# ZhenghaoFei/visual_odom

Measured on NVIDIA B200. Metric: stereo frames/sec at 1241x376, 2000 feats; LK kernel HBM GB/s vs roofline, higher is better.
Workload: dtype u8/i32 fixed point + f32 (LK), f64 (pose)

## Files before the change

### visual_odom_b200/csrc/batch.cu

```cuda
#include "ctx.h"
#include <string.h>

__global__ void k_pack_counts(vo_unit_result_dev* res, const int* n_pts, const int* n_det, const int* n3, const int* n5,
                              int n_units, int detect)
{
    const int u = blockIdx.x * blockDim.x + threadIdx.x;
    if (u >= n_units) return;
    res[u].n_features = n_pts[u];
    res[u].n_detected = detect ? n_det[u] : 0;
    res[u].n_tracked = n3[u];
    res[u].n_valid = n5[u];
}

#define VO_OUT_BYTES_PER_SLOT (4 * sizeof(float2) + sizeof(int) + sizeof(float3) + sizeof(int))
__global__ void k_pack_outputs(uint8_t* __restrict__ out, size_t stride, int per, const float2* __restrict__ valid4, size_t cs,
                               const int* __restrict__ idx5, const float3* __restrict__ X, const int* __restrict__ inliers,
                               const int* __restrict__ n5, const vo_unit_result_dev* __restrict__ res, int cap)
{
    const int u = blockIdx.x;
    const int nv = min(n5[u], per), ni = min(res[u].n_inliers, per);
    float2* o4 = reinterpret_cast<float2*>(out + (size_t)u * stride);
    int* ok = reinterpret_cast<int*>(o4 + 4 * (size_t)per);
    float* oX = reinterpret_cast<float*>(ok + per);
    int* oi = reinterpret_cast<int*>(oX + 3 * (size_t)per);
// ... 125 lines not shown
    return VO_OK;
}

static int ensure_hi_streams(vo_ctx* ctx)
{
    if (ctx->hi_stream[0]) return VO_OK;
    int lo = 0, hi = 0;
    VO_CUDA_CHECK(cudaDeviceGetStreamPriorityRange(&lo, &hi));
    for (int c = 0; c < VO_LANES; c++) {
        VO_CUDA_CHECK(cudaStreamCreateWithPriority(&ctx->hi_stream[c], cudaStreamNonBlocking, hi));
        for (int k = 0; k < 4; k++) VO_CUDA_CHECK(cudaEventCreateWithFlags(&ctx->hi_ev[c][k], cudaEventDisableTiming));
    }
    return VO_OK;
}

static int run_range_launch(vo_ctx* ctx, const View& v)
{
    ctx->imgs_per_unit = 4;
    int rc;
    int c = -1;
    for (int k = 0; k < VO_LANES; k++) if (ctx->side_stream[k] && v.s == ctx->side_stream[k]) c = k;
    const bool part = ctx->part_on && c >= 0;
    const bool prio = !part && ctx->use_priorities && c >= 0;
    View h = v, lk = v;
    cudaEvent_t* ev = nullptr;
    if (part) {
        h.s = ctx->part_hp_stream[c]; lk.s = ctx->part_lk_stream[c]; ev = ctx->part_ev[c];
    } else if (prio) {
        if ((rc = ensure_hi_streams(ctx))) return rc;
        h.s = ctx->hi_stream[c]; ev = ctx->hi_ev[c];
    }
    View pre = h;
    if (part && ctx->part_pre_with_lk) pre.s = lk.s;
    if (ev) {
        VO_CUDA_CHECK(cudaEventRecord(ev[0], v.s));
        VO_CUDA_CHECK(cudaStreamWaitEvent(pre.s, ev[0], 0));
        if (pre.s != h.s) VO_CUDA_CHECK(cudaStreamWaitEvent(h.s, ev[0], 0));
    }
    if (ctx->batch_detect) {
        if ((rc = vo_run_fast(ctx, pre, 0, false))) return rc;
        if ((rc = vo_run_select(ctx, pre))) return rc;
    }
    if ((rc = vo_run_pyramid(ctx, v.u0 * ctx->imgs_per_unit, v.n * ctx->imgs_per_unit, pre.s))) return rc;
    if (ev && pre.s != lk.s) {
        VO_CUDA_CHECK(cudaEventRecord(ev[1], pre.s));
        VO_CUDA_CHECK(cudaStreamWaitEvent(lk.s, ev[1], 0));
    }
    const int ip[4] = {0, 1, 3, 2}, in[4] = {1, 3, 2, 0};
    ctx->lk_per_unit = ctx->batch_max_pts;
    rc = vo_run_lk_ring(ctx, lk, 4, ip, in, false);
    ctx->lk_per_unit = 0;
    if (rc) return rc;
    if (ev) {
        VO_CUDA_CHECK(cudaEventRecord(ev[2], lk.s));
        VO_CUDA_CHECK(cudaStreamWaitEvent(h.s, ev[2], 0));
    }
    if ((rc = vo_run_filter(ctx, h, false))) return rc;
    const size_t cs = (size_t)ctx->units * ctx->cap;
    if ((rc = vo_run_triangulate(ctx, h, ctx->d_valid4, ctx->d_valid4 + cs, ctx->d_n5))) return rc;
    float K9[9] = {ctx->P_l[0], ctx->P_l[1], ctx->P_l[2], ctx->P_l[4], ctx->P_l[5], ctx->P_l[6], ctx->P_l[8], ctx->P_l[9], ctx->P_l[10]};
    if ((rc = vo_run_pnp(ctx, h, ctx->d_valid4 + 2 * cs, ctx->d_n5, K9))) return rc;
    k_pack_counts<<<(v.n + 63) / 64, 64, 0, h.s>>>(ctx->d_results + v.u0, ctx->d_npts + v.u0, ctx->d_ndet + v.u0, ctx->d_n3 + v.u0,
                                                  ctx->d_n5 + v.u0, v.n, ctx->batch_detect ? 1 : 0);
    ctx->launches += 1;
    VO_CUDA_CHECK(cudaGetLastError());
    if (ev) {
        VO_CUDA_CHECK(cudaEventRecord(ev[3], h.s));
        VO_CUDA_CHECK(cudaStreamWaitEvent(v.s, ev[3], 0));
    }
    return VO_OK;
}

static int run_range(vo_ctx* ctx, const View& v)
{
    bool on_side = false;
    for (int k = 0; k < VO_LANES; k++) on_side = on_side || (ctx->side_stream[k] && v.s == ctx->side_stream[k]);
// ... 237 lines not shown
```

### visual_odom_b200/csrc/ctx.cu

```cuda
#include "ctx.h"
#include <string.h>
#include <stdlib.h>

void vo_set_error(vo_ctx* ctx, const char* fmt, ...)
{
    if (!ctx) return;
    va_list ap;
    va_start(ap, fmt);
    vsnprintf(ctx->err, sizeof(ctx->err), fmt, ap);
    va_end(ap);
}

extern "C" void vo_default_params(vo_params* p)
{
    p->fast_threshold = 20;
    p->fast_nonmax = 1;
    p->lk_win = 21;
    p->lk_max_level = 3;
    p->lk_max_iters = 30;
    p->lk_epsilon = 0.01;
    p->lk_min_eig = 0.001;
    p->circ_threshold = 0;
    p->pnp_iterations = 500;
    p->pnp_reproj_error = 0.5f;
// ... 155 lines not shown
    if (!allow_pending_batches)
        for (auto& p : ctx->pending)
            if (p.active) {
                vo_set_error(ctx, "%s: the vo_batch_submit submission of slots [%d, %d) has not been waited for", who, p.u0, p.u0 + p.n);
                return VO_E_INVALID;
            }
    ctx->seq_active = false;
    return VO_OK;
}

typedef CUresult (*PFN_cuDeviceGet)(CUdevice*, int);
typedef CUresult (*PFN_cuDeviceGetDevResource)(CUdevice, CUdevResource*, CUdevResourceType);
typedef CUresult (*PFN_cuDevSmResourceSplitByCount)(CUdevResource*, unsigned int*, const CUdevResource*, CUdevResource*, unsigned int, unsigned int);
typedef CUresult (*PFN_cuDevResourceGenerateDesc)(CUdevResourceDesc*, CUdevResource*, unsigned int);
typedef CUresult (*PFN_cuGreenCtxCreate)(CUgreenCtx*, CUdevResourceDesc, CUdevice, unsigned int);
typedef CUresult (*PFN_cuGreenCtxStreamCreate)(CUstream*, CUgreenCtx, unsigned int, int);
typedef CUresult (*PFN_cuGreenCtxDestroy)(CUgreenCtx);

template <typename F>
static bool drv(const char* name, F* fn)
{
    void* p = nullptr;
    cudaDriverEntryPointQueryResult q;
    if (cudaGetDriverEntryPoint(name, &p, cudaEnableDefault, &q) != cudaSuccess || q != cudaDriverEntryPointSuccess || !p) return false;
    *fn = (F)p;
    return true;
}

void vo_partition_destroy(vo_ctx* ctx)
{
    for (int c = 0; c < VO_LANES; c++) {
        if (ctx->part_lk_stream[c]) cudaStreamDestroy(ctx->part_lk_stream[c]);
        if (ctx->part_hp_stream[c]) cudaStreamDestroy(ctx->part_hp_stream[c]);
        ctx->part_lk_stream[c] = ctx->part_hp_stream[c] = nullptr;
        for (int k = 0; k < 4; k++) if (ctx->part_ev[c][k]) { cudaEventDestroy(ctx->part_ev[c][k]); ctx->part_ev[c][k] = nullptr; }
    }
    PFN_cuGreenCtxDestroy destroy = nullptr;
    if (drv("cuGreenCtxDestroy", &destroy))
        for (int k = 0; k < 2; k++) if (ctx->part_gctx[k]) destroy((CUgreenCtx)ctx->part_gctx[k]);
    ctx->part_gctx[0] = ctx->part_gctx[1] = nullptr;
    ctx->part_on = false; ctx->part_helper_sms = ctx->part_lk_sms = 0;
}

int vo_partition_enable(vo_ctx* ctx, int helper_sms)
{
    VO_CUDA_CHECK(cudaSetDevice(ctx->device));
    int rc = vo_drain_pending(ctx);
    if (rc) return rc;
    VO_CUDA_CHECK(cudaDeviceSynchronize());
    vo_drop_graphs(ctx);
    vo_partition_destroy(ctx);
    if (helper_sms <= 0) return VO_OK;
    PFN_cuDeviceGet dget; PFN_cuDeviceGetDevResource getres; PFN_cuDevSmResourceSplitByCount split;
    PFN_cuDevResourceGenerateDesc gendesc; PFN_cuGreenCtxCreate create; PFN_cuGreenCtxStreamCreate screate;
    if (!drv("cuDeviceGet", &dget) || !drv("cuDeviceGetDevResource", &getres) || !drv("cuDevSmResourceSplitByCount", &split) ||
        !drv("cuDevResourceGenerateDesc", &gendesc) || !drv("cuGreenCtxCreate", &create) || !drv("cuGreenCtxStreamCreate", &screate)) {
        vo_set_error(ctx, "sm_partition: this driver has no green-context API");
        return VO_E_UNSUPPORTED;
    }
    CUdevice dev;
    CUdevResource all, part[1], rest;
    unsigned int nb = 1;
    CUresult r;
    if ((r = dget(&dev, ctx->device)) != CUDA_SUCCESS || (r = getres(dev, &all, CU_DEV_RESOURCE_TYPE_SM)) != CUDA_SUCCESS ||
        (r = split(part, &nb, &all, &rest, 0, (unsigned)helper_sms)) != CUDA_SUCCESS || nb != 1) {
        vo_set_error(ctx, "sm_partition: splitting off %d SMs failed (driver error %d)", helper_sms, (int)r);
        return VO_E_UNSUPPORTED;
    }
    CUdevResource* rs[2] = {&part[0], &rest};
    for (int k = 0; k < 2; k++) {
        CUdevResourceDesc desc;
        CUgreenCtx g;
        if ((r = gendesc(&desc, rs[k], 1)) != CUDA_SUCCESS || (r = create(&g, desc, dev, CU_GREEN_CTX_DEFAULT_STREAM)) != CUDA_SUCCESS) {
            vo_set_error(ctx, "sm_partition: cuGreenCtxCreate failed (driver error %d)", (int)r);
            vo_partition_destroy(ctx);
            return VO_E_UNSUPPORTED;
        }
        ctx->part_gctx[k] = g;
    }
    ctx->part_helper_sms = (int)part[0].sm.smCount; ctx->part_lk_sms = (int)rest.sm.smCount;
    for (int c = 0; c < VO_LANES; c++) {
        CUstream a, b;
        if ((r = screate(&a, (CUgreenCtx)ctx->part_gctx[0], CU_STREAM_NON_BLOCKING, 0)) != CUDA_SUCCESS ||
            (r = screate(&b, (CUgreenCtx)ctx->part_gctx[1], CU_STREAM_NON_BLOCKING, 0)) != CUDA_SUCCESS) {
            vo_set_error(ctx, "sm_partition: cuGreenCtxStreamCreate failed (driver error %d)", (int)r);
            vo_partition_destroy(ctx);
            return VO_E_UNSUPPORTED;
        }
        ctx->part_hp_stream[c] = (cudaStream_t)a; ctx->part_lk_stream[c] = (cudaStream_t)b;
        for (int k = 0; k < 4; k++) VO_CUDA_CHECK(cudaEventCreateWithFlags(&ctx->part_ev[c][k], cudaEventDisableTiming));
    }
    ctx->part_on = true;
    return VO_OK;
}

int vo_drain_pending(vo_ctx* ctx)
{
    for (auto& p : ctx->pending)
        if (p.active) {
            VO_CUDA_CHECK(cudaEventSynchronize(p.done));
            p.active = false;
        }
    if (ctx->seq_inflight > 0 && ctx->side_stream[0]) VO_CUDA_CHECK(cudaStreamSynchronize(ctx->side_stream[0]));
    return VO_OK;
}

void vo_drop_graphs(vo_ctx* ctx)
{
    for (auto& g : ctx->graphs) cudaGraphExecDestroy(g.exec);
    ctx->graphs.clear();
}

void vo_set_calibration(vo_ctx* ctx, const float P_l[12], const float P_r[12])
{
    const bool same = ctx->have_P && memcmp(ctx->P_l, P_l, 12 * sizeof(float)) == 0 && memcmp(ctx->P_r, P_r, 12 * sizeof(float)) == 0;
    if (same) return;
    vo_drop_graphs(ctx);
    memcpy(ctx->P_l, P_l, 12 * sizeof(float));
    memcpy(ctx->P_r, P_r, 12 * sizeof(float));
    ctx->have_P = true;
}

void vo_free_state(vo_ctx* ctx)
// ... 235 lines not shown
        for (int c = 0; c < VO_LANES; c++) if (ctx->part_on && v.s == ctx->part_lk_stream[c]) lk_sms = ctx->part_lk_sms;
        VO_CUDA_CHECK(vo_launch_lk_ring(ctx->maps, a, lk_sms, ctx->lk_ctas_per_sm, v.s));
    }
    ctx->launches += 1;
    if (e1) VO_CUDA_CHECK(cudaEventRecord(e1, v.s));
    return VO_OK;
}

int vo_run_filter(vo_ctx* ctx, const View& v, bool with_ages)
{
    const size_t uo = (size_t)v.u0 * ctx->cap;
    FilterArgs f;
    memset(&f, 0, sizeof(f));
    f.cap = ctx->cap;
    f.call_stride = (size_t)ctx->units * ctx->cap;
    f.circ_threshold = ctx->p.circ_threshold;
    f.n_pts = ctx->d_npts + v.u0;
    f.pts_in = ctx->d_pts_in + uo;
    f.pts_out = ctx->d_pts_out + uo;
    f.status = ctx->d_status + uo;
    f.ages_in = with_ages ? ctx->d_ages_in + uo : nullptr;
    f.ages_out = ctx->d_ages_out + uo;
    f.kept5 = ctx->d_kept5 + uo;
    f.idx3 = ctx->d_idx3 + uo;
    f.n3 = ctx->d_n3 + v.u0;
    f.valid4 = ctx->d_valid4 + uo;
    f.idx5 = ctx->d_idx5 + uo;
    f.n5 = ctx->d_n5 + v.u0;
    VO_CUDA_CHECK(vo_launch_ring_filter(f, v.n, v.s));
    ctx->launches += 1;
    return VO_OK;
}

int vo_run_fast(vo_ctx* ctx, const View& v, int plane_in_unit, bool want_resp)
{
    FastArgs a;
    memset(&a, 0, sizeof(a));
    const size_t plane = (size_t)ctx->w * ctx->h;
    a.n_units = v.n;
    a.img_tab = ctx->d_raw_tab + (size_t)(v.plane0 >= 0 ? v.plane0 : v.u0 * ctx->imgs_per_unit) + plane_in_unit;
    a.img_stride_idx = ctx->imgs_per_unit;
    a.w = ctx->w; a.h = ctx->h; a.pitch = ctx->w;
    a.threshold = ctx->p.fast_threshold; a.nonmax = ctx->p.fast_nonmax;
    a.score = ctx->d_score + v.u0 * plane; a.score_plane = plane;
    a.rowbuf = ctx->d_rowbuf + v.u0 * plane; a.rowcap = ctx->w;
    a.rowcount = ctx->d_rowcount + (size_t)v.u0 * ctx->h; a.rowoff = ctx->d_rowoff + (size_t)v.u0 * ctx->h;
    a.n_det = ctx->d_ndet + v.u0;
    a.corners = ctx->d_corners + (size_t)v.u0 * ctx->corner_cap;
    a.resp = want_resp ? ctx->d_resp + (size_t)v.u0 * ctx->corner_cap : nullptr;
    a.corner_cap = ctx->corner_cap;
    ctx->launches += vo_launch_fast(a, v.s);
    VO_CUDA_CHECK(cudaGetLastError());
    return VO_OK;
}

int vo_run_select(vo_ctx* ctx, const View& v)
{
    ctx->launches += vo_launch_select(ctx->d_corners + (size_t)v.u0 * ctx->corner_cap, ctx->corner_cap, ctx->d_ndet + v.u0,
                                      ctx->d_want + v.u0, ctx->d_pts_in + (size_t)v.u0 * ctx->cap, ctx->cap, ctx->d_npts + v.u0,
                                      v.n, v.s);
    VO_CUDA_CHECK(cudaGetLastError());
    return VO_OK;
}

int vo_run_triangulate(vo_ctx* ctx, const View& v, const float2* pts_l, const float2* pts_r, const int* n, float4* X4)
{
    const size_t uo = (size_t)v.u0 * ctx->cap;
    TriArgs t;
    memset(&t, 0, sizeof(t));
    t.cap = ctx->cap; t.n_pts = n + v.u0; t.pts_l = pts_l + uo; t.pts_r = pts_r + uo; t.X = ctx->d_X + uo; t.X4 = X4;
    for (int k = 0; k < 12; k++) { t.Pl[k] = (double)ctx->P_l[k]; t.Pr[k] = (double)ctx->P_r[k]; }
    ctx->launches += vo_launch_triangulate(t, v.n, v.s);
    VO_CUDA_CHECK(cudaGetLastError());
    return VO_OK;
}

int vo_run_pnp(vo_ctx* ctx, const View& v, const float2* pts2d, const int* n, const float* K9)
{
    const size_t uo = (size_t)v.u0 * ctx->cap, its = (size_t)ctx->p.pnp_iterations;
    PnpArgs a;
    memset(&a, 0, sizeof(a));
    a.n_units = v.n; a.cap = ctx->cap; a.iterations = ctx->p.pnp_iterations;
    a.n_pts = n + v.u0; a.X = ctx->d_X + uo; a.x = pts2d + uo;
    a.fu = (double)K9[0]; a.fv = (double)K9[4]; a.uc = (double)K9[2]; a.vc = (double)K9[5];
    const double thr = (double)ctx->p.pnp_reproj_error;
    a.thr2 = (float)(thr * thr);
    a.confidence = ctx->p.pnp_confidence;
    a.t_prev = ctx->d_tprev + (size_t)v.u0 * 3;
    a.state = ctx->d_pnp_state + v.u0; a.subsets = ctx->d_subsets + v.u0 * its * 5; a.models = ctx->d_models + v.u0 * its * 12;
    a.counts = ctx->d_counts + v.u0 * its;
    a.inliers = ctx->d_inliers + uo; a.results = ctx->d_results + v.u0;
    ctx->launches += vo_launch_pnp(a, v.s);
    VO_CUDA_CHECK(cudaGetLastError());
    return VO_OK;
// ... 2 lines not shown
```

### visual_odom_b200/csrc/ctx.h

```cpp
#pragma once
#include "common.cuh"
#include "lk_ring.h"
#include "filter.h"
#include "fast.h"
#include "pnp.h"
#include "seq.h"
#include "ess.h"
#include "../../include/vo_b200.h"
#include <vector>
#include <stdarg.h>
#define LK_QUEUES 32
#define VO_DIST_BUCKET 4
#define VO_DIST_NB 4
#define VO_LANES 3

struct vo_ctx {
    int device = 0;
    cudaStream_t own_stream = nullptr, stream = nullptr;
    vo_params p;
    char err[1024] = {0};
    long long launches = 0;
    int sm_count = 0;

    int w = 0, h = 0;
// ... 30 lines not shown
    int* d_want = nullptr;
    int corner_cap = 0;
    float3* d_X = nullptr;
    double* d_tprev = nullptr;
    PnpState* d_pnp_state = nullptr;
    int* d_subsets = nullptr;
    double* d_models = nullptr;
    int* d_counts = nullptr;
    int* d_inliers = nullptr;
    vo_unit_result_dev* d_results = nullptr;
    float2* d_feat_pts = nullptr;
    int* d_feat_ages = nullptr;
    int* d_feat_cnt = nullptr;
    int* d_bucket = nullptr;
    int* d_seq_err = nullptr;
    int feat_cap = 0, bucket_cap = 4096;
    bool seq_active = false;
    int seq_slot = 0;
    int seq_inflight = 0;
    long long seq_submitted = 0;
    int seq_channels[2] = {1, 1};
    cudaEvent_t seq_front_ev[2] = {nullptr, nullptr}, seq_back_ev[2] = {nullptr, nullptr};
    long long seq_frames = 0;
    double seq_pose[16] = {1,0,0,0, 0,1,0,0, 0,0,1,0, 0,0,0,1};
    uint8_t* d_bgr = nullptr;
    size_t bgr_bytes = 0;
    bool part_on = false;
    bool part_auto = true;
    bool part_pre_with_lk = false;
    int part_helper_sms = 0, part_lk_sms = 0;
    void* part_gctx[2] = {nullptr, nullptr};
    cudaStream_t part_lk_stream[VO_LANES] = {};
    cudaStream_t part_hp_stream[VO_LANES] = {};
    cudaEvent_t part_ev[VO_LANES][4] = {};
    void* dist_comm = nullptr;
    int dist_rank = 0, dist_world = 1;
    cudaStream_t dist_stream = nullptr, dist_snap_stream = nullptr;
    struct DistBucket { void* d = nullptr; void* h = nullptr; cudaEvent_t done = nullptr; int fill = 0, unwaited = 0, n_units = 0; bool flushed = false; };
    struct DistStep { int bucket = 0, index = 0; };
    DistBucket dist_bk[VO_DIST_NB];
    DistStep dist_steps[2 * VO_DIST_DEPTH];
    int dist_cur = 0;
    cudaEvent_t dist_ev_read = nullptr, dist_ev_fork = nullptr;
    size_t dist_bytes = 0;
    long long dist_head = 0, dist_tail = 0;
    void* d_ess = nullptr;
    int ess_cap = 0;
    std::vector<void*> allocs;

    void* h_pinned = nullptr;
    size_t h_pinned_bytes = 0;

    std::vector<cudaEvent_t> ev_pool;
    size_t ev_used = 0;
    double lk_ms = 0.0;
    long long lk_n = 0;
    bool lk_timing = true;
    bool lk_use_tma = true;
    int lk_ctas_per_sm = 0;
    int lk_quota = 0;
    int lk_span = 0;
    int* d_lk_progress = nullptr;
    int lk_per_unit = 0;
    int* d_lk_queue = nullptr;
    std::vector<cudaStream_t> lk_queue_streams;

    int batch_units = 0;
// ... 11 lines not shown
    cudaStream_t side_stream[VO_LANES] = {};
    cudaEvent_t fork_ev = nullptr, join_ev[VO_LANES] = {};
    struct Pending { int u0 = 0, n = 0; bool active = false; cudaEvent_t done = nullptr; };
    std::vector<Pending> pending;
    bool batch_outputs = false;
    uint8_t* d_out = nullptr;
    uint8_t* h_out = nullptr;
    size_t out_stride = 0;
    int out_per = 0, out_units = 0;
    unsigned submit_count = 0;
};

void vo_set_error(vo_ctx* ctx, const char* fmt, ...);
int vo_ensure_state(vo_ctx* ctx, int w, int h, int units, int imgs_per_unit);
void vo_free_state(vo_ctx* ctx);
void vo_drop_graphs(vo_ctx* ctx);
void vo_set_calibration(vo_ctx* ctx, const float P_l[12], const float P_r[12]);
int vo_drain_pending(vo_ctx* ctx);
int vo_partition_enable(vo_ctx* ctx, int helper_sms);
void vo_partition_destroy(vo_ctx* ctx);
int vo_dist_order_after_gathers(vo_ctx* ctx, cudaStream_t st);
void vo_dist_shutdown(vo_ctx* ctx);
int vo_claim_buffers(vo_ctx* ctx, const char* who, bool allow_pending_batches = false);
int vo_ensure_pinned(vo_ctx* ctx, size_t bytes);
int vo_ensure_bgr(vo_ctx* ctx, size_t bytes);
int vo_launch_bgr_to_gray(const uint8_t* d_bgr, size_t pitch, size_t img_stride_in, uint8_t* d_gray, size_t img_stride_out,
                          int w, int h, int n_img, cudaStream_t s);
struct View { int u0, n; cudaStream_t s; int plane0 = -1; };
int vo_run_lk(vo_ctx* ctx, const View& v, int ncalls, const int* img_prev, const int* img_next, bool want_err);
int vo_run_pyramid(vo_ctx* ctx, int plane0, int nplanes, cudaStream_t s);
int vo_run_lk_ring(vo_ctx* ctx, const View& v, int ncalls, const int* img_prev, const int* img_next, bool want_err);
int vo_run_filter(vo_ctx* ctx, const View& v, bool with_ages);
int vo_run_fast(vo_ctx* ctx, const View& v, int plane_in_unit, bool want_resp);
int vo_run_select(vo_ctx* ctx, const View& v);
int vo_run_triangulate(vo_ctx* ctx, const View& v, const float2* pts_l, const float2* pts_r, const int* n, float4* X4 = nullptr);
int vo_run_pnp(vo_ctx* ctx, const View& v, const float2* pts2d, const int* n, const float* K9);
```

### visual_odom_b200/csrc/fast.cu

```cuda
#include "common.cuh"
#include "fast.h"

__constant__ int c_ring_dx[16] = {0, 1, 2, 3, 3, 3, 2, 1, 0, -1, -2, -3, -3, -3, -2, -1};
__constant__ int c_ring_dy[16] = {3, 3, 2, 1, 0, -1, -2, -3, -3, -3, -2, -1, 0, 1, 2, 3};

__global__ void __launch_bounds__(256) k_fast_score(const uint8_t* const* __restrict__ img_tab, int img_stride_idx,
                                                    int w, int h, int pitch, int threshold,
                                                    uint8_t* __restrict__ score, size_t score_plane)
{
    const int unit = blockIdx.z;
    const uint8_t* __restrict__ img = img_tab[unit * img_stride_idx];
    uint8_t* __restrict__ sc = score + (size_t)unit * score_plane;
    const int x = blockIdx.x * 32 + (threadIdx.x & 31);
    const int y = blockIdx.y * 8 + (threadIdx.x >> 5);
    if (x >= w || y >= h) return;
    int result = 0;
    if (x >= 3 && x < w - 3 && y >= 3 && y < h - 3) {
        const uint8_t* p = img + (size_t)y * pitch + x;
        const int v = p[0];
        int d[16];
        unsigned hi = 0, lo = 0;
#pragma unroll
        for (int k = 0; k < 16; k++) {
            const int r = p[c_ring_dy[k] * pitch + c_ring_dx[k]];
            d[k] = v - r;
            hi |= (unsigned)(r > v + threshold) << k;
            lo |= (unsigned)(r < v - threshold) << k;
        }
        unsigned mh = hi | (hi << 16), ml = lo | (lo << 16);
        mh &= mh >> 1; mh &= mh >> 2; mh &= mh >> 4; mh &= mh >> 1;
        ml &= ml >> 1; ml &= ml >> 2; ml &= ml >> 4; ml &= ml >> 1;
        if (mh | ml) {
            int mn[16], mx[16];
#pragma unroll
            for (int k = 0; k < 16; k++) { mn[k] = min(d[k], d[(k + 1) & 15]); mx[k] = max(d[k], d[(k + 1) & 15]); }
            int mn4[16], mx4[16];
#pragma unroll
            for (int k = 0; k < 16; k++) { mn4[k] = min(mn[k], mn[(k + 2) & 15]); mx4[k] = max(mx[k], mx[(k + 2) & 15]); }
            int A = -1000, B = 1000;
#pragma unroll
            for (int k = 0; k < 16; k++) {
                int a8 = min(mn4[k], mn4[(k + 4) & 15]);
                int b8 = max(mx4[k], mx4[(k + 4) & 15]);
                A = max(A, min(a8, d[(k + 8) & 15]));
                B = min(B, max(b8, d[(k + 8) & 15]));
            }
            result = max(threshold, max(A, -B)) - 1;
        }
    }
    sc[(size_t)y * w + x] = (uint8_t)result;
}

#define NMS_T 256
#define NMS_NC 8
__global__ void __launch_bounds__(NMS_T) k_fast_nms_row(const uint8_t* __restrict__ score, size_t score_plane, int w, int h,
                                                        int nonmax, uint16_t* __restrict__ rowbuf, int rowcap,
                                                        int* __restrict__ rowcount)
{
    const int y = blockIdx.x, unit = blockIdx.y;
    const uint8_t* __restrict__ sc = score + (size_t)unit * score_plane;
    uint16_t* __restrict__ out = rowbuf + ((size_t)unit * h + y) * rowcap;
    __shared__ uint8_t rows[3][NMS_T * NMS_NC + 2];
    __shared__ int wcnt[NMS_NC * (NMS_T / 32)];
    __shared__ int base;
    if (y < 3 || y >= h - 3) {
        if (threadIdx.x == 0) rowcount[unit * h + y] = 0;
        return;
    }
    if (threadIdx.x == 0) base = 0;
    const int lane = threadIdx.x & 31, warp = threadIdx.x >> 5;
    constexpr int NW = NMS_T / 32, SPAN = NMS_T * NMS_NC;
    for (int x0 = 0; x0 < w; x0 += SPAN) {
        for (int i = threadIdx.x; i < SPAN + 2; i += NMS_T) {
            const int x = x0 - 1 + i;
            const bool in = (x >= 0 && x < w);
            rows[0][i] = in ? sc[(size_t)(y - 1) * w + x] : 0;
            rows[1][i] = in ? sc[(size_t)y * w + x] : 0;
            rows[2][i] = in ? sc[(size_t)(y + 1) * w + x] : 0;
        }
        __syncthreads();
        unsigned bal[NMS_NC];
#pragma unroll
        for (int c = 0; c < NMS_NC; c++) {
            const int x = x0 + c * NMS_T + threadIdx.x, i = c * NMS_T + threadIdx.x + 1;
            bool keep = false;
            if (x < w) {
                const int s = rows[1][i];
                if (s > 0) {
                    keep = !nonmax ||
                           (s > rows[1][i - 1] && s > rows[1][i + 1] && s > rows[0][i - 1] && s > rows[0][i] &&
                            s > rows[0][i + 1] && s > rows[2][i - 1] && s > rows[2][i] && s > rows[2][i + 1]);
                }
            }
            bal[c] = __ballot_sync(0xffffffffu, keep);
            if (lane == 0) wcnt[c * NW + warp] = __popc(bal[c]);
        }
        __syncthreads();
        int carry_total = 0;
        if (threadIdx.x < NMS_NC * NW) {
            const int v = wcnt[threadIdx.x];
            int incl = v;
#pragma unroll
            for (int d = 1; d < 32; d <<= 1) {
                const int o = __shfl_up_sync(0xffffffffu, incl, d);
                if (lane >= d) incl += o;
            }
            carry_total = incl;
            wcnt[threadIdx.x] = incl - v;
        }
        __shared__ int w0_total, pass_total;
        if (threadIdx.x == 31) w0_total = carry_total;
        __syncthreads();
        if (threadIdx.x >= 32 && threadIdx.x < NMS_NC * NW) wcnt[threadIdx.x] += w0_total;
        if (threadIdx.x == NMS_NC * NW - 1) pass_total = carry_total + w0_total;
        __syncthreads();
        const int b0 = base;
#pragma unroll
        for (int c = 0; c < NMS_NC; c++) {
            if ((bal[c] >> lane) & 1u) {
                const int o = b0 + wcnt[c * NW + warp] + __popc(bal[c] & ((1u << lane) - 1u));
                if (o < rowcap) out[o] = (uint16_t)(x0 + c * NMS_T + threadIdx.x);
            }
        }
        __syncthreads();
        if (threadIdx.x == 0) base = b0 + pass_total;
        __syncthreads();
    }
    if (threadIdx.x == 0) rowcount[unit * h + y] = base < rowcap ? base : rowcap;
}

__global__ void __launch_bounds__(1024) k_fast_scan(const int* __restrict__ rowcount, int h, int* __restrict__ rowoff,
                                                    int* __restrict__ n_det)
{
    const int unit = blockIdx.x;
    const int* rc = rowcount + unit * h;
    int* ro = rowoff + unit * h;
    __shared__ int wsum[32];
    __shared__ int carry;
    if (threadIdx.x == 0) carry = 0;
    __syncthreads();
    const int lane = threadIdx.x & 31, warp = threadIdx.x >> 5;
    for (int y0 = 0; y0 < h; y0 += 1024) {
        const int y = y0 + threadIdx.x;
        int v = (y < h) ? rc[y] : 0;
        int incl = v;
#pragma unroll
        for (int d = 1; d < 32; d <<= 1) {
            int o = __shfl_up_sync(0xffffffffu, incl, d);
            if (lane >= d) incl += o;
        }
        if (lane == 31) wsum[warp] = incl;
        __syncthreads();
        int woff = carry;
        for (int k = 0; k < warp; k++) woff += wsum[k];
        if (y < h) ro[y] = woff + incl - v;
        __syncthreads();
        if (threadIdx.x == 0) {
            int t = 0;
            for (int k = 0; k < 32; k++) t += wsum[k];
            carry += t;
        }
        __syncthreads();
    }
    if (threadIdx.x == 0) n_det[unit] = carry;
}

__global__ void __launch_bounds__(128) k_fast_gather(const uint16_t* __restrict__ rowbuf, int rowcap,
                                                     const int* __restrict__ rowcount, const int* __restrict__ rowoff,
                                                     int h, const uint8_t* __restrict__ score, size_t score_plane, int w,
                                                     float2* __restrict__ out, float* __restrict__ resp, int cap)
{
    const int y = blockIdx.x, unit = blockIdx.y;
    const int n = rowcount[unit * h + y], off = rowoff[unit * h + y];
    const uint16_t* src = rowbuf + ((size_t)unit * h + y) * rowcap;
    for (int i = threadIdx.x; i < n; i += blockDim.x) {
        const int o = off + i;
        if (o < cap) {
            const int x = src[i];
            out[(size_t)unit * cap + o] = make_float2((float)x, (float)y);
            if (resp) resp[(size_t)unit * cap + o] = (float)score[(size_t)unit * score_plane + (size_t)y * w + x];
        }
    }
}

__global__ void k_select_stride(const float2* __restrict__ corners, int corner_cap, const int* __restrict__ n_det,
                                const int* __restrict__ want, float2* __restrict__ pts, int cap, int* __restrict__ n_pts)
{
    const int unit = blockIdx.y;
    int m = n_det[unit];
    if (m > corner_cap) m = corner_cap;
    int n = want[unit];
    if (n > cap) n = cap;
    if (n > m) n = m;
    const int i = blockIdx.x * blockDim.x + threadIdx.x;
    if (i == 0) n_pts[unit] = n;
    if (i >= n) return;
    const long idx = (n > 1) ? ((long)i * (m - 1)) / (n - 1) : 0;
    pts[(size_t)unit * cap + i] = corners[(size_t)unit * corner_cap + idx];
}

int vo_launch_fast(const FastArgs& a, cudaStream_t stream)
{
    dim3 g1((a.w + 31) / 32, (a.h + 7) / 8, a.n_units);
    k_fast_score<<<g1, 256, 0, stream>>>(a.img_tab, a.img_stride_idx, a.w, a.h, a.pitch, a.threshold, a.score, a.score_plane);
    dim3 g2(a.h, a.n_units);
    k_fast_nms_row<<<g2, NMS_T, 0, stream>>>(a.score, a.score_plane, a.w, a.h, a.nonmax, a.rowbuf, a.rowcap, a.rowcount);
    k_fast_scan<<<a.n_units, 1024, 0, stream>>>(a.rowcount, a.h, a.rowoff, a.n_det);
    k_fast_gather<<<g2, 128, 0, stream>>>(a.rowbuf, a.rowcap, a.rowcount, a.rowoff, a.h, a.score, a.score_plane, a.w,
                                           a.corners, a.resp, a.corner_cap);
    return 4;
}

int vo_launch_select(const float2* corners, int corner_cap, const int* n_det, const int* want, float2* pts, int cap,
                     int* n_pts, int n_units, cudaStream_t stream)
{
    dim3 g((cap + 255) / 256, n_units);
    k_select_stride<<<g, 256, 0, stream>>>(corners, corner_cap, n_det, want, pts, cap, n_pts);
    return 1;
}
```

### visual_odom_b200/csrc/fast.h

```cpp
#pragma once
#include "common.cuh"

struct FastArgs {
    int n_units;
    const uint8_t* const* img_tab;
    int img_stride_idx;
    int w, h, pitch;
    int threshold, nonmax;
    uint8_t* score;
    size_t score_plane;
    uint16_t* rowbuf;
    int rowcap;
    int* rowcount;
    int* rowoff;
    int* n_det;
    float2* corners;
    float* resp;
    int corner_cap;
};

int vo_launch_fast(const FastArgs& a, cudaStream_t stream);
int vo_launch_select(const float2* corners, int corner_cap, const int* n_det, const int* want, float2* pts, int cap,
                     int* n_pts, int n_units, cudaStream_t stream);
```

Measured before the change: 4652.

## Fuse FAST scoring, NMS and selection into shared-memory kernels on separate streams

Replaces the separate FAST score, row-NMS, scan, gather and stride-select kernels with one shared-memory tiled detect kernel. It uses SIMD byte compares to find candidates, scores them per warp, and does NMS with ballot compaction in place. A new select kernel scans row counts and binary-searches rows, which skips the corner gather and scan passes. In partitioned mode, detection can also run on dedicated fast streams, chosen by an env var, that overlap with the pyramid build and join LK through an extra event. This cuts the number of launches and the global score-map traffic, at the cost of more complexity and an undocumented env-var switch.

```diff
diff --git a/visual_odom_b200/csrc/batch.cu b/visual_odom_b200/csrc/batch.cu
--- a/visual_odom_b200/csrc/batch.cu
+++ b/visual_odom_b200/csrc/batch.cu
@@ -181,16 +181,28 @@
     }
     View pre = h;
     if (part && ctx->part_pre_with_lk) pre.s = lk.s;
+    View fs = pre;
+    if (part && ctx->part_pre_with_lk && ctx->batch_detect) {
+        bool others = false;
+        for (auto& p : ctx->pending) others = others || p.active;
+        const char* x = getenv("VO_X");
+        const int mode = x ? atoi(x) : 2;
+        if (mode == 0) fs.s = ctx->part_fast_stream[c];
+        else if (mode == 1) fs.s = ctx->part_fast_hp_stream[c];
+        else if (mode == 2) fs.s = others ? ctx->part_fast_hp_stream[c] : ctx->part_fast_stream[c];
+    }
     if (ev) {
         VO_CUDA_CHECK(cudaEventRecord(ev[0], v.s));
         VO_CUDA_CHECK(cudaStreamWaitEvent(pre.s, ev[0], 0));
         if (pre.s != h.s) VO_CUDA_CHECK(cudaStreamWaitEvent(h.s, ev[0], 0));
-    }
-    if (ctx->batch_detect) {
-        if ((rc = vo_run_fast(ctx, pre, 0, false))) return rc;
-        if ((rc = vo_run_select(ctx, pre))) return rc;
-    }
+        if (fs.s != pre.s) VO_CUDA_CHECK(cudaStreamWaitEvent(fs.s, ev[0], 0));
+    }
+    if (ctx->batch_detect && (rc = vo_run_fast_select(ctx, fs))) return rc;
     if ((rc = vo_run_pyramid(ctx, v.u0 * ctx->imgs_per_unit, v.n * ctx->imgs_per_unit, pre.s))) return rc;
+    if (fs.s != pre.s) {
+        VO_CUDA_CHECK(cudaEventRecord(ev[4], fs.s));
+        VO_CUDA_CHECK(cudaStreamWaitEvent(lk.s, ev[4], 0));
+    }
     if (ev && pre.s != lk.s) {
         VO_CUDA_CHECK(cudaEventRecord(ev[1], pre.s));
         VO_CUDA_CHECK(cudaStreamWaitEvent(lk.s, ev[1], 0));
diff --git a/visual_odom_b200/csrc/ctx.cu b/visual_odom_b200/csrc/ctx.cu
--- a/visual_odom_b200/csrc/ctx.cu
+++ b/visual_odom_b200/csrc/ctx.cu
@@ -211,8 +211,10 @@
     for (int c = 0; c < VO_LANES; c++) {
         if (ctx->part_lk_stream[c]) cudaStreamDestroy(ctx->part_lk_stream[c]);
         if (ctx->part_hp_stream[c]) cudaStreamDestroy(ctx->part_hp_stream[c]);
-        ctx->part_lk_stream[c] = ctx->part_hp_stream[c] = nullptr;
-        for (int k = 0; k < 4; k++) if (ctx->part_ev[c][k]) { cudaEventDestroy(ctx->part_ev[c][k]); ctx->part_ev[c][k] = nullptr; }
+        if (ctx->part_fast_stream[c]) cudaStreamDestroy(ctx->part_fast_stream[c]);
+        if (ctx->part_fast_hp_stream[c]) cudaStreamDestroy(ctx->part_fast_hp_stream[c]);
+        ctx->part_lk_stream[c] = ctx->part_hp_stream[c] = ctx->part_fast_stream[c] = ctx->part_fast_hp_stream[c] = nullptr;
+        for (int k = 0; k < 5; k++) if (ctx->part_ev[c][k]) { cudaEventDestroy(ctx->part_ev[c][k]); ctx->part_ev[c][k] = nullptr; }
     }
     PFN_cuGreenCtxDestroy destroy = nullptr;
     if (drv("cuGreenCtxDestroy", &destroy))
@@ -259,15 +261,18 @@
     }
     ctx->part_helper_sms = (int)part[0].sm.smCount; ctx->part_lk_sms = (int)rest.sm.smCount;
     for (int c = 0; c < VO_LANES; c++) {
-        CUstream a, b;
+        CUstream a, b, f, fh;
         if ((r = screate(&a, (CUgreenCtx)ctx->part_gctx[0], CU_STREAM_NON_BLOCKING, 0)) != CUDA_SUCCESS ||
-            (r = screate(&b, (CUgreenCtx)ctx->part_gctx[1], CU_STREAM_NON_BLOCKING, 0)) != CUDA_SUCCESS) {
+            (r = screate(&b, (CUgreenCtx)ctx->part_gctx[1], CU_STREAM_NON_BLOCKING, 0)) != CUDA_SUCCESS ||
+            (r = screate(&f, (CUgreenCtx)ctx->part_gctx[1], CU_STREAM_NON_BLOCKING, 0)) != CUDA_SUCCESS ||
+            (r = screate(&fh, (CUgreenCtx)ctx->part_gctx[0], CU_STREAM_NON_BLOCKING, 0)) != CUDA_SUCCESS) {
             vo_set_error(ctx, "sm_partition: cuGreenCtxStreamCreate failed (driver error %d)", (int)r);
             vo_partition_destroy(ctx);
             return VO_E_UNSUPPORTED;
         }
-        ctx->part_hp_stream[c] = (cudaStream_t)a; ctx->part_lk_stream[c] = (cudaStream_t)b;
-        for (int k = 0; k < 4; k++) VO_CUDA_CHECK(cudaEventCreateWithFlags(&ctx->part_ev[c][k], cudaEventDisableTiming));
+        ctx->part_hp_stream[c] = (cudaStream_t)a; ctx->part_lk_stream[c] = (cudaStream_t)b; ctx->part_fast_stream[c] = (cudaStream_t)f;
+        ctx->part_fast_hp_stream[c] = (cudaStream_t)fh;
+        for (int k = 0; k < 5; k++) VO_CUDA_CHECK(cudaEventCreateWithFlags(&ctx->part_ev[c][k], cudaEventDisableTiming));
     }
     ctx->part_on = true;
     return VO_OK;
@@ -569,7 +574,7 @@
     return VO_OK;
 }
 
-int vo_run_fast(vo_ctx* ctx, const View& v, int plane_in_unit, bool want_resp)
+static FastArgs fast_args(vo_ctx* ctx, const View& v, int plane_in_unit, bool want_resp)
 {
     FastArgs a;
     memset(&a, 0, sizeof(a));
@@ -586,17 +591,25 @@
     a.corners = ctx->d_corners + (size_t)v.u0 * ctx->corner_cap;
     a.resp = want_resp ? ctx->d_resp + (size_t)v.u0 * ctx->corner_cap : nullptr;
     a.corner_cap = ctx->corner_cap;
-    ctx->launches += vo_launch_fast(a, v.s);
+    return a;
+}
+
+int vo_run_fast(vo_ctx* ctx, const View& v, int plane_in_unit, bool want_resp)
+{
+    const int n = vo_launch_fast(fast_args(ctx, v, plane_in_unit, want_resp), v.s);
     VO_CUDA_CHECK(cudaGetLastError());
-    return VO_OK;
-}
-
-int vo_run_select(vo_ctx* ctx, const View& v)
-{
-    ctx->launches += vo_launch_select(ctx->d_corners + (size_t)v.u0 * ctx->corner_cap, ctx->corner_cap, ctx->d_ndet + v.u0,
-                                      ctx->d_want + v.u0, ctx->d_pts_in + (size_t)v.u0 * ctx->cap, ctx->cap, ctx->d_npts + v.u0,
-                                      v.n, v.s);
+    if (n < 0) { vo_set_error(ctx, "FAST detector: shared memory for %d-pixel rows not granted", ctx->w); return VO_E_CUDA; }
+    ctx->launches += n;
+    return VO_OK;
+}
+
+int vo_run_fast_select(vo_ctx* ctx, const View& v)
+{
+    const int n = vo_launch_fast_select(fast_args(ctx, v, 0, false), ctx->d_want + v.u0, ctx->d_pts_in + (size_t)v.u0 * ctx->cap,
+                                        ctx->cap, ctx->d_npts + v.u0, v.s);
     VO_CUDA_CHECK(cudaGetLastError());
+    if (n < 0) { vo_set_error(ctx, "FAST detector / selection: shared memory for a %dx%d image not granted", ctx->w, ctx->h); return VO_E_CUDA; }
+    ctx->launches += n;
     return VO_OK;
 }
 
diff --git a/visual_odom_b200/csrc/ctx.h b/visual_odom_b200/csrc/ctx.h
--- a/visual_odom_b200/csrc/ctx.h
+++ b/visual_odom_b200/csrc/ctx.h
@@ -86,7 +86,9 @@
     void* part_gctx[2] = {nullptr, nullptr};
     cudaStream_t part_lk_stream[VO_LANES] = {};
     cudaStream_t part_hp_stream[VO_LANES] = {};
-    cudaEvent_t part_ev[VO_LANES][4] = {};
+    cudaStream_t part_fast_stream[VO_LANES] = {};
+    cudaStream_t part_fast_hp_stream[VO_LANES] = {};
+    cudaEvent_t part_ev[VO_LANES][5] = {};
     void* dist_comm = nullptr;
     int dist_rank = 0, dist_world = 1;
     cudaStream_t dist_stream = nullptr, dist_snap_stream = nullptr;
@@ -164,6 +166,6 @@
 int vo_run_lk_ring(vo_ctx* ctx, const View& v, int ncalls, const int* img_prev, const int* img_next, bool want_err);
 int vo_run_filter(vo_ctx* ctx, const View& v, bool with_ages);
 int vo_run_fast(vo_ctx* ctx, const View& v, int plane_in_unit, bool want_resp);
-int vo_run_select(vo_ctx* ctx, const View& v);
+int vo_run_fast_select(vo_ctx* ctx, const View& v);
 int vo_run_triangulate(vo_ctx* ctx, const View& v, const float2* pts_l, const float2* pts_r, const int* n, float4* X4 = nullptr);
 int vo_run_pnp(vo_ctx* ctx, const View& v, const float2* pts2d, const int* n, const float* K9);
diff --git a/visual_odom_b200/csrc/fast.cu b/visual_odom_b200/csrc/fast.cu
--- a/visual_odom_b200/csrc/fast.cu
+++ b/visual_odom_b200/csrc/fast.cu
@@ -4,129 +4,202 @@
 __constant__ int c_ring_dx[16] = {0, 1, 2, 3, 3, 3, 2, 1, 0, -1, -2, -3, -3, -3, -2, -1};
 __constant__ int c_ring_dy[16] = {3, 3, 2, 1, 0, -1, -2, -3, -3, -3, -2, -1, 0, 1, 2, 3};
 
-__global__ void __launch_bounds__(256) k_fast_score(const uint8_t* const* __restrict__ img_tab, int img_stride_idx,
-                                                    int w, int h, int pitch, int threshold,
-                                                    uint8_t* __restrict__ score, size_t score_plane)
-{
-    const int unit = blockIdx.z;
+static __device__ __forceinline__ bool fast_arc9(unsigned m)
+{
+    m |= m << 16;
+    m &= m >> 1; m &= m >> 2; m &= m >> 4; m &= m >> 1;
+    return m != 0;
+}
+
+static __device__ __forceinline__ int fast_score(const int d[16], int threshold)
+{
+    int mn[16], mx[16];
+#pragma unroll
+    for (int k = 0; k < 16; k++) { mn[k] = min(d[k], d[(k + 1) & 15]); mx[k] = max(d[k], d[(k + 1) & 15]); }
+    int mn4[16], mx4[16];
+#pragma unroll
+    for (int k = 0; k < 16; k++) { mn4[k] = min(mn[k], mn[(k + 2) & 15]); mx4[k] = max(mx[k], mx[(k + 2) & 15]); }
+    int A = -1000, B = 1000;
+#pragma unroll
+    for (int k = 0; k < 16; k++) {
+        int a8 = min(mn4[k], mn4[(k + 4) & 15]);
+        int b8 = max(mx4[k], mx4[(k + 4) & 15]);
+        A = max(A, min(a8, d[(k + 8) & 15]));
+        B = min(B, max(b8, d[(k + 8) & 15]));
+    }
+    return max(threshold, max(A, -B)) - 1;
+}
+
+#define FD_T 256
+#define FD_ROWS (FD_T / 32)
+#define FD_SPAN 2048
+#define FD_IROWS (FD_ROWS + 8)
+#define FD_QCAP (4 * 32 + 32)
+
+struct FdGeom {
+    int rows;
+    int groups;
+    int iw;
+    int ss;
+    __host__ __device__ FdGeom(int span, int rows_) : rows(rows_)
+    {
+        groups = (span + 2 + 3) / 4;
+        iw = groups + 5;
+        ss = 4 * groups;
+    }
+    __host__ __device__ size_t bytes() const
+    {
+        return (size_t)(rows + 8) * iw * 4 + (size_t)(rows + 2) * ss + FD_IROWS * 4 + (size_t)(FD_T / 32) * FD_QCAP * 4;
+    }
+};
+
+__global__ void __launch_bounds__(FD_T) k_fast_detect(const uint8_t* const* __restrict__ img_tab, int img_stride_idx,
+                                                       int w, int h, int pitch, int threshold, int nonmax, int span, int rows,
+                                                       uint8_t* __restrict__ score, size_t score_plane,
+                                                       uint16_t* __restrict__ rowbuf, int rowcap, int* __restrict__ rowcount)
+{
+    extern __shared__ __align__(16) uint32_t fd_smem[];
+    const int unit = blockIdx.y, y0 = blockIdx.x * rows;
+    const int lane = threadIdx.x & 31, warp = threadIdx.x >> 5;
     const uint8_t* __restrict__ img = img_tab[unit * img_stride_idx];
-    uint8_t* __restrict__ sc = score + (size_t)unit * score_plane;
-    const int x = blockIdx.x * 32 + (threadIdx.x & 31);
-    const int y = blockIdx.y * 8 + (threadIdx.x >> 5);
-    if (x >= w || y >= h) return;
-    int result = 0;
-    if (x >= 3 && x < w - 3 && y >= 3 && y < h - 3) {
-        const uint8_t* p = img + (size_t)y * pitch + x;
-        const int v = p[0];
-        int d[16];
-        unsigned hi = 0, lo = 0;
-#pragma unroll
-        for (int k = 0; k < 16; k++) {
-            const int r = p[c_ring_dy[k] * pitch + c_ring_dx[k]];
-            d[k] = v - r;
-            hi |= (unsigned)(r > v + threshold) << k;
-            lo |= (unsigned)(r < v - threshold) << k;
-        }
-        unsigned mh = hi | (hi << 16), ml = lo | (lo << 16);
-        mh &= mh >> 1; mh &= mh >> 2; mh &= mh >> 4; mh &= mh >> 1;
-        ml &= ml >> 1; ml &= ml >> 2; ml &= ml >> 4; ml &= ml >> 1;
-        if (mh | ml) {
-            int mn[16], mx[16];
-#pragma unroll
-            for (int k = 0; k < 16; k++) { mn[k] = min(d[k], d[(k + 1) & 15]); mx[k] = max(d[k], d[(k + 1) & 15]); }
-            int mn4[16], mx4[16];
-#pragma unroll
-            for (int k = 0; k < 16; k++) { mn4[k] = min(mn[k], mn[(k + 2) & 15]); mx4[k] = max(mx[k], mx[(k + 2) & 15]); }
-            int A = -1000, B = 1000;
-#pragma unroll
-            for (int k = 0; k < 16; k++) {
-                int a8 = min(mn4[k], mn4[(k + 4) & 15]);
-                int b8 = max(mx4[k], mx4[(k + 4) & 15]);
-                A = max(A, min(a8, d[(k + 8) & 15]));
-                B = min(B, max(b8, d[(k + 8) & 15]));
-            }
-            result = max(threshold, max(A, -B)) - 1;
-        }
-    }
-    sc[(size_t)y * w + x] = (uint8_t)result;
-}
-
-#define NMS_T 256
-#define NMS_NC 8
-__global__ void __launch_bounds__(NMS_T) k_fast_nms_row(const uint8_t* __restrict__ score, size_t score_plane, int w, int h,
-                                                        int nonmax, uint16_t* __restrict__ rowbuf, int rowcap,
-                                                        int* __restrict__ rowcount)
-{
-    const int y = blockIdx.x, unit = blockIdx.y;
-    const uint8_t* __restrict__ sc = score + (size_t)unit * score_plane;
-    uint16_t* __restrict__ out = rowbuf + ((size_t)unit * h + y) * rowcap;
-    __shared__ uint8_t rows[3][NMS_T * NMS_NC + 2];
-    __shared__ int wcnt[NMS_NC * (NMS_T / 32)];
-    __shared__ int base;
-    if (y < 3 || y >= h - 3) {
-        if (threadIdx.x == 0) rowcount[unit * h + y] = 0;
-        return;
-    }
-    if (threadIdx.x == 0) base = 0;
-    const int lane = threadIdx.x & 31, warp = threadIdx.x >> 5;
-    constexpr int NW = NMS_T / 32, SPAN = NMS_T * NMS_NC;
-    for (int x0 = 0; x0 < w; x0 += SPAN) {
-        for (int i = threadIdx.x; i < SPAN + 2; i += NMS_T) {
-            const int x = x0 - 1 + i;
-            const bool in = (x >= 0 && x < w);
-            rows[0][i] = in ? sc[(size_t)(y - 1) * w + x] : 0;
-            rows[1][i] = in ? sc[(size_t)y * w + x] : 0;
-            rows[2][i] = in ? sc[(size_t)(y + 1) * w + x] : 0;
-        }
-        __syncthreads();
-        unsigned bal[NMS_NC];
-#pragma unroll
-        for (int c = 0; c < NMS_NC; c++) {
-            const int x = x0 + c * NMS_T + threadIdx.x, i = c * NMS_T + threadIdx.x + 1;
-            bool keep = false;
-            if (x < w) {
-                const int s = rows[1][i];
-                if (s > 0) {
-                    keep = !nonmax ||
-                           (s > rows[1][i - 1] && s > rows[1][i + 1] && s > rows[0][i - 1] && s > rows[0][i] &&
-                            s > rows[0][i + 1] && s > rows[2][i - 1] && s > rows[2][i] && s > rows[2][i + 1]);
-                }
-            }
-            bal[c] = __ballot_sync(0xffffffffu, keep);
-            if (lane == 0) wcnt[c * NW + warp] = __popc(bal[c]);
-        }
-        __syncthreads();
-        int carry_total = 0;
-        if (threadIdx.x < NMS_NC * NW) {
-            const int v = wcnt[threadIdx.x];
-            int incl = v;
+    const FdGeom G(span, rows);
+    uint32_t* s_img = fd_smem;
+    uint8_t* s_sc = reinterpret_cast<uint8_t*>(s_img + (rows + 8) * G.iw);
+    int* s_sh = reinterpret_cast<int*>(s_sc + (rows + 2) * G.ss);
+    int* q = s_sh + FD_IROWS + warp * FD_QCAP;
+    const uint8_t* s_b = reinterpret_cast<const uint8_t*>(s_img);
+    const uint32_t t4 = 0x01010101u * (uint32_t)threshold;
+    int base = 0;
+
+    for (int x0 = 0; x0 < w; x0 += span) {
+        const int c0 = x0 - 4;
+        for (int t = threadIdx.x; t < (rows + 8) * G.iw; t += FD_T) {
+            const int i = t / G.iw, k = t - i * G.iw, Y = y0 - 4 + i;
+            uint32_t v = 0;
+            int sh = 0;
+            if (Y >= 0 && Y < h) {
+                const uint8_t* p = img + (size_t)Y * pitch;
+                const uintptr_t a = (uintptr_t)p + (intptr_t)c0;
+                sh = (int)(a & 3u);
+                const long col = (long)(a - sh - (uintptr_t)p) + 4L * k;
+                if (col >= 0 && col + 4 <= w) {
+                    v = __ldg(reinterpret_cast<const uint32_t*>(p + col));
+                } else {
+#pragma unroll
+                    for (int b = 0; b < 4; b++)
+                        if (col + b >= 0 && col + b < w) v |= (uint32_t)__ldg(p + col + b) << (8 * b);
+                }
+            }
+            s_img[t] = v;
+            if (k == 0) s_sh[i] = sh;
+        }
+        __syncthreads();
+
+        const int ntask = (rows + 2) * G.groups;
+        int qn = 0;
+        for (int tb = warp * 32; tb < ntask; tb += FD_T) {
+            const int t = tb + lane;
+            unsigned cand = 0;
+            int sr = 0, g = 0;
+            if (t < ntask) {
+                sr = t / G.groups; g = t - sr * G.groups;
+                reinterpret_cast<uint32_t*>(s_sc + sr * G.ss)[g] = 0;
+                const int y = y0 - 1 + sr, x = x0 - 1 + 4 * g;
+                if (y >= 3 && y < h - 3 && x + 3 >= 3 && x < w - 3) {
+                    auto ld4 = [&](int ir, int c) {
+                        const int o = s_sh[ir] + (c - c0);
+                        const uint32_t* r = s_img + ir * G.iw + (o >> 2);
+                        return __funnelshift_r(r[0], r[1], 8 * (o & 3));
+                    };
+                    const uint32_t v = ld4(sr + 3, x);
+                    const uint32_t vhi = __vaddus4(v, t4), vlo = __vsubus4(v, t4);
+                    uint32_t hi0 = 0, hi1 = 0, lo0 = 0, lo1 = 0;
+#pragma unroll
+                    for (int k = 0; k < 16; k++) {
+                        const uint32_t r = ld4(sr + 3 + c_ring_dy[k], x + c_ring_dx[k]);
+                        const uint32_t bh = (__vcmpgtu4(r, vhi) & 0x01010101u) << (k & 7);
+                        const uint32_t bl = (__vcmpltu4(r, vlo) & 0x01010101u) << (k & 7);
+                        if (k < 8) { hi0 |= bh; lo0 |= bl; } else { hi1 |= bh; lo1 |= bl; }
+                    }
+#pragma unroll
+                    for (int i = 0; i < 4; i++) {
+                        const unsigned mh = ((hi0 >> (8 * i)) & 255u) | (((hi1 >> (8 * i)) & 255u) << 8);
+                        const unsigned ml = ((lo0 >> (8 * i)) & 255u) | (((lo1 >> (8 * i)) & 255u) << 8);
+                        if (x + i >= 3 && x + i < w - 3 && (fast_arc9(mh) || fast_arc9(ml))) cand |= 1u << i;
+                    }
+                }
+            }
+            const int nc = __popc(cand);
+            int incl = nc;
 #pragma unroll
             for (int d = 1; d < 32; d <<= 1) {
                 const int o = __shfl_up_sync(0xffffffffu, incl, d);
                 if (lane >= d) incl += o;
             }
-            carry_total = incl;
-            wcnt[threadIdx.x] = incl - v;
-        }
-        __shared__ int w0_total, pass_total;
-        if (threadIdx.x == 31) w0_total = carry_total;
-        __syncthreads();
-        if (threadIdx.x >= 32 && threadIdx.x < NMS_NC * NW) wcnt[threadIdx.x] += w0_total;
-        if (threadIdx.x == NMS_NC * NW - 1) pass_total = carry_total + w0_total;
-        __syncthreads();
-        const int b0 = base;
-#pragma unroll
-        for (int c = 0; c < NMS_NC; c++) {
-            if ((bal[c] >> lane) & 1u) {
-                const int o = b0 + wcnt[c * NW + warp] + __popc(bal[c] & ((1u << lane) - 1u));
-                if (o < rowcap) out[o] = (uint16_t)(x0 + c * NMS_T + threadIdx.x);
-            }
-        }
-        __syncthreads();
-        if (threadIdx.x == 0) base = b0 + pass_total;
-        __syncthreads();
-    }
-    if (threadIdx.x == 0) rowcount[unit * h + y] = base < rowcap ? base : rowcap;
+            int o = qn + incl - nc;
+            for (unsigned m = cand; m; m &= m - 1) q[o++] = (sr << 16) | (4 * g + __ffs(m) - 1);
+            qn += __shfl_sync(0xffffffffu, incl, 31);
+            __syncwarp();
+            while (qn >= 32) {
+                qn -= 32;
+                const int e = q[qn + lane];
+                __syncwarp();
+                const int r = e >> 16, c = e & 0xffff;
+                const uint8_t* ctr = s_b + (r + 3) * G.iw * 4 + s_sh[r + 3] + (x0 - 1 + c - c0);
+                const int p = *ctr;
+                int d[16];
+#pragma unroll
+                for (int k = 0; k < 16; k++) {
+                    const int rr = r + 3 + c_ring_dy[k];
+                    d[k] = p - (int)s_b[rr * G.iw * 4 + s_sh[rr] + (x0 - 1 + c + c_ring_dx[k] - c0)];
+                }
+                s_sc[r * G.ss + c] = (uint8_t)fast_score(d, threshold);
+            }
+        }
+        if (lane < qn) {
+            const int e = q[lane];
+            const int r = e >> 16, c = e & 0xffff;
+            const int p = s_b[(r + 3) * G.iw * 4 + s_sh[r + 3] + (x0 - 1 + c - c0)];
+            int d[16];
+#pragma unroll
+            for (int k = 0; k < 16; k++) {
+                const int rr = r + 3 + c_ring_dy[k];
+                d[k] = p - (int)s_b[rr * G.iw * 4 + s_sh[rr] + (x0 - 1 + c + c_ring_dx[k] - c0)];
+            }
+            s_sc[r * G.ss + c] = (uint8_t)fast_score(d, threshold);
+        }
+        __syncthreads();
+
+        const int y = y0 + warp;
+        if (warp < rows && y < h) {
+            const uint8_t* s0 = s_sc + warp * G.ss;
+            const uint8_t* s1 = s0 + G.ss;
+            const uint8_t* s2 = s1 + G.ss;
+            uint16_t* __restrict__ out = rowbuf + ((size_t)unit * h + y) * rowcap;
+            uint8_t* __restrict__ sc = score + (size_t)unit * score_plane + (size_t)y * w;
+            const int xe = min(w, x0 + span);
+            for (int xb = x0; xb < xe; xb += 32) {
+                const int x = xb + lane, i = x - x0 + 1;
+                bool keep = false;
+                int s = 0;
+                if (x < xe) {
+                    s = s1[i];
+                    keep = s > 0 && (!nonmax || (s > s1[i - 1] && s > s1[i + 1] && s > s0[i - 1] && s > s0[i] &&
+                                                  s > s0[i + 1] && s > s2[i - 1] && s > s2[i] && s > s2[i + 1]));
+                }
+                const unsigned bal = __ballot_sync(0xffffffffu, keep);
+                if (keep) {
+                    const int o = base + __popc(bal & ((1u << lane) - 1u));
+                    if (o < rowcap) out[o] = (uint16_t)x;
+                    sc[x] = (uint8_t)s;
+                }
+                base += __popc(bal);
+            }
+        }
+        __syncthreads();
+    }
+    const int y = y0 + warp;
+    if (lane == 0 && warp < rows && y < h) rowcount[unit * h + y] = base < rowcap ? base : rowcap;
 }
 
 __global__ void __launch_bounds__(1024) k_fast_scan(const int* __restrict__ rowcount, int h, int* __restrict__ rowoff,
@@ -183,38 +256,105 @@
     }
 }
 
-__global__ void k_select_stride(const float2* __restrict__ corners, int corner_cap, const int* __restrict__ n_det,
-                                const int* __restrict__ want, float2* __restrict__ pts, int cap, int* __restrict__ n_pts)
-{
-    const int unit = blockIdx.y;
-    int m = n_det[unit];
-    if (m > corner_cap) m = corner_cap;
+#define SEL_T 1024
+__global__ void __launch_bounds__(SEL_T) k_select_rows(const uint16_t* __restrict__ rowbuf, int rowcap,
+                                                       const int* __restrict__ rowcount, int h, int corner_cap,
+                                                       int* __restrict__ n_det, const int* __restrict__ want,
+                                                       float2* __restrict__ pts, int cap, int* __restrict__ n_pts)
+{
+    extern __shared__ int s_inc[];
+    __shared__ int wsum[SEL_T / 32];
+    __shared__ int carry;
+    const int unit = blockIdx.x;
+    const int* rc = rowcount + unit * h;
+    const int lane = threadIdx.x & 31, warp = threadIdx.x >> 5;
+    if (threadIdx.x == 0) carry = 0;
+    __syncthreads();
+    for (int y0 = 0; y0 < h; y0 += SEL_T) {
+        const int y = y0 + threadIdx.x;
+        int incl = (y < h) ? rc[y] : 0;
+#pragma unroll
+        for (int d = 1; d < 32; d <<= 1) {
+            const int o = __shfl_up_sync(0xffffffffu, incl, d);
+            if (lane >= d) incl += o;
+        }
+        if (lane == 31) wsum[warp] = incl;
+        __syncthreads();
+        int woff = carry;
+        for (int k = 0; k < warp; k++) woff += wsum[k];
+        if (y < h) s_inc[y] = woff + incl;
+        __syncthreads();
+        if (threadIdx.x == 0) {
+            int t = 0;
+            for (int k = 0; k < SEL_T / 32; k++) t += wsum[k];
+            carry += t;
+        }
+        __syncthreads();
+    }
+    const int total = carry;
+    const int m = total < corner_cap ? total : corner_cap;
     int n = want[unit];
     if (n > cap) n = cap;
     if (n > m) n = m;
-    const int i = blockIdx.x * blockDim.x + threadIdx.x;
-    if (i == 0) n_pts[unit] = n;
-    if (i >= n) return;
-    const long idx = (n > 1) ? ((long)i * (m - 1)) / (n - 1) : 0;
-    pts[(size_t)unit * cap + i] = corners[(size_t)unit * corner_cap + idx];
+    if (threadIdx.x == 0) { n_det[unit] = total; n_pts[unit] = n; }
+    for (int i = threadIdx.x; i < n; i += SEL_T) {
+        const int idx = (n > 1) ? (int)(((long)i * (m - 1)) / (n - 1)) : 0;
+        int lo = 0, hi = h - 1;
+        while (lo < hi) {
+            const int mid = (lo + hi) >> 1;
+            if (s_inc[mid] > idx) hi = mid; else lo = mid + 1;
+        }
+        const int k = idx - (s_inc[lo] - rc[lo]);
+        pts[(size_t)unit * cap + i] = make_float2((float)rowbuf[((size_t)unit * h + lo) * rowcap + k], (float)lo);
+    }
+}
+
+static int launch_detect(const FastArgs& a, cudaStream_t stream)
+{
+    const int passes = (a.w + FD_SPAN - 1) / FD_SPAN, span = (a.w + passes - 1) / passes;
+    static int sms = 0;
+    if (!sms) {
+        int dev = 0;
+        if (cudaGetDevice(&dev) != cudaSuccess || cudaDeviceGetAttribute(&sms, cudaDevAttrMultiProcessorCount, dev) != cudaSuccess) return -1;
+    }
+    int rows = FD_ROWS;
+    while (rows > 1 && (long)a.n_units * ((a.h + rows - 1) / rows) < sms) rows >>= 1;
+    const size_t smem = FdGeom(span, rows).bytes();
+    static size_t smem_set = 48 * 1024;
+    if (smem > smem_set) {
+        const size_t most = FdGeom(FD_SPAN, FD_ROWS).bytes();
+        if (cudaFuncSetAttribute(k_fast_detect, cudaFuncAttributeMaxDynamicSharedMemorySize, (int)most) != cudaSuccess) return -1;
+        smem_set = most;
+    }
+    const int thr = a.threshold < 0 ? 0 : (a.threshold > 255 ? 255 : a.threshold);
+    dim3 g((a.h + rows - 1) / rows, a.n_units);
+    k_fast_detect<<<g, FD_T, smem, stream>>>(a.img_tab, a.img_stride_idx, a.w, a.h, a.pitch, thr, a.nonmax, span, rows,
+                                              a.score, a.score_plane, a.rowbuf, a.rowcap, a.rowcount);
+    return 1;
 }
 
 int vo_launch_fast(const FastArgs& a, cudaStream_t stream)
 {
-    dim3 g1((a.w + 31) / 32, (a.h + 7) / 8, a.n_units);
-    k_fast_score<<<g1, 256, 0, stream>>>(a.img_tab, a.img_stride_idx, a.w, a.h, a.pitch, a.threshold, a.score, a.score_plane);
+    const int n = launch_detect(a, stream);
+    if (n < 0) return n;
+    k_fast_scan<<<a.n_units, 1024, 0, stream>>>(a.rowcount, a.h, a.rowoff, a.n_det);
     dim3 g2(a.h, a.n_units);
-    k_fast_nms_row<<<g2, NMS_T, 0, stream>>>(a.score, a.score_plane, a.w, a.h, a.nonmax, a.rowbuf, a.rowcap, a.rowcount);
-    k_fast_scan<<<a.n_units, 1024, 0, stream>>>(a.rowcount, a.h, a.rowoff, a.n_det);
     k_fast_gather<<<g2, 128, 0, stream>>>(a.rowbuf, a.rowcap, a.rowcount, a.rowoff, a.h, a.score, a.score_plane, a.w,
                                            a.corners, a.resp, a.corner_cap);
-    return 4;
-}
-
-int vo_launch_select(const float2* corners, int corner_cap, const int* n_det, const int* want, float2* pts, int cap,
-                     int* n_pts, int n_units, cudaStream_t stream)
-{
-    dim3 g((cap + 255) / 256, n_units);
-    k_select_stride<<<g, 256, 0, stream>>>(corners, corner_cap, n_det, want, pts, cap, n_pts);
-    return 1;
-}
+    return n + 2;
+}
+
+int vo_launch_fast_select(const FastArgs& a, const int* want, float2* pts, int cap, int* n_pts, cudaStream_t stream)
+{
+    const int n = launch_detect(a, stream);
+    if (n < 0) return n;
+    const size_t smem = (size_t)a.h * sizeof(int);
+    static size_t smem_set = 48 * 1024;
+    if (smem > smem_set) {
+        if (cudaFuncSetAttribute(k_select_rows, cudaFuncAttributeMaxDynamicSharedMemorySize, (int)smem) != cudaSuccess) return -1;
+        smem_set = smem;
+    }
+    k_select_rows<<<a.n_units, SEL_T, smem, stream>>>(a.rowbuf, a.rowcap, a.rowcount, a.h, a.corner_cap, a.n_det, want, pts,
+                                                       cap, n_pts);
+    return n + 1;
+}
diff --git a/visual_odom_b200/csrc/fast.h b/visual_odom_b200/csrc/fast.h
--- a/visual_odom_b200/csrc/fast.h
+++ b/visual_odom_b200/csrc/fast.h
@@ -20,5 +20,4 @@
 };
 
 int vo_launch_fast(const FastArgs& a, cudaStream_t stream);
-int vo_launch_select(const float2* corners, int corner_cap, const int* n_det, const int* want, float2* pts, int cap,
-                     int* n_pts, int n_units, cudaStream_t stream);
+int vo_launch_fast_select(const FastArgs& a, const int* want, float2* pts, int cap, int* n_pts, cudaStream_t stream);
```

New measurement: 3112, median of 6. -33.1%, worse.
